# LinXueyuanStdio/LaTeX_OCR

Hardware: NVIDIA H100
Metric: formula-images/sec (train step, 128x512 px, seq<=150) (higher is better)
Workload: dtype bf16

## Files before the change

### latex_ocr_b200/csrc/lo_attention.cu

```cuda
#include <cooperative_groups.h>

#include "lo_common.cuh"
#include "lo_ptx.cuh"

namespace cg = cooperative_groups;

namespace lo {

#ifndef LO_ATT_RPW
#define LO_ATT_RPW 2
#endif
#ifndef LO_ATT_MINB
#define LO_ATT_MINB 2
#endif
#define AP_THREADS 288
#define AP_CWARPS 8
#define AP_STAGES 3
#define AP_MAXSPLIT 16


#ifdef LO_ATT_TIMING
__device__ long long* g_att_ts = nullptr;
__device__ __forceinline__ void att_ts(int k) {
  if (g_att_ts) {
    long long t;
    asm volatile("mov.u64 %0, %%globaltimer;" : "=l"(t));
    g_att_ts[((int64_t)blockIdx.y * gridDim.x + blockIdx.x) * 16 + k] = t;
  }
}
#define ATT_TS(k, cond) do { if (cond) att_ts(k); } while (0)
#else
#define ATT_TS(k, cond) do { } while (0)
#endif

__device__ __forceinline__ uint64_t make_policy(int kind) {
  return kind == 1 ? l2_policy_evict_last() : (kind == 2 ? l2_policy_evict_first() : l2_policy_evict_normal());
}

template <int ACT, bool APPROX>
__device__ __forceinline__ float att_act(float x) {
  if constexpr (ACT == 0) return fmaxf(x, 0.f);
  else if constexpr (APPROX) {
    float y;
    asm("tanh.approx.f32 %0, %1;" : "=f"(y) : "f"(x));
    return y;
  } else return tanhf(x);
}
template <int ACT>
__device__ __forceinline__ float att_dact(float pre, float post) {
  if constexpr (ACT == 0) return pre > 0.f ? 1.f : 0.f;
  else return 1.f - post * post;
}

__host__ __device__ __forceinline__ int att_rows_per_split(int R, int nsplit) { return (((R + nsplit - 1) / nsplit) + 1) & ~1; }

template <typename T, int NVA, int NVC>
struct ApCfg {
  static constexpr int CHA = NVA * 256;
  static constexpr int CHC = NVC * 256;
  static constexpr int NVM = NVA > NVC ? NVA : NVC;
  static constexpr int RPW = (sizeof(T) == 2 && NVM <= 2) ? LO_ATT_RPW : 1;
  static constexpr int ROWS = AP_CWARPS * RPW;
  static constexpr int HALF_A = ROWS * CHA;
  static constexpr int HALF_C = ROWS * CHC;
  static constexpr int STAGE_ELEMS = HALF_A + HALF_C;
  static constexpr int STAGE_BYTES = STAGE_ELEMS * (int)sizeof(T);
  static constexpr int SMEM = AP_STAGES * STAGE_BYTES + 128;
};

template <typename T, int NVA, int NVC, bool CL, int ACT, bool MK>
__global__ void __launch_bounds__(AP_THREADS, LO_ATT_MINB) attention_fwd_pipe_kernel(
    const T* __restrict__ att1, const T* __restrict__ enc, const float* __restrict__ att2, int64_t att2_stride,
    const float* __restrict__ wf, float* __restrict__ alpha, int64_t alpha_stride, float* __restrict__ ctx,
    float* __restrict__ gate_pre, int64_t gate_stride, float* __restrict__ gctx, bf16* __restrict__ gctx_bf, int R, int nsplit,
    int* __restrict__ counters, float* __restrict__ partials, int pol_enc, int pol_att1, int rpi, uint8_t* __restrict__ mask_out) {
  using C = ApCfg<T, NVA, NVC>;
  constexpr int CHA = C::CHA, CHC = C::CHC;
  extern __shared__ __align__(128) uint8_t ap_smem[];
  T* ring = reinterpret_cast<T*>(ap_smem);
  uint64_t* full_bar = reinterpret_cast<uint64_t*>(ap_smem + AP_STAGES * C::STAGE_BYTES);
  uint64_t* empty_bar = full_bar + AP_STAGES;
  float* s_e = reinterpret_cast<float*>(ap_smem + AP_STAGES * C::STAGE_BYTES + 128);
  __shared__ float s_m[AP_CWARPS], s_l[AP_CWARPS];
  __shared__ float s_scale[AP_MAXSPLIT];
  __shared__ float s_ML[2];
  __shared__ int s_last;

  const int b = blockIdx.y, sp = blockIdx.x;
  const int lane = threadIdx.x & 31, wid = threadIdx.x >> 5;
  const int rps = (R + nsplit - 1) / nsplit;
  const int r0 = sp * rps, r1 = min(R, r0 + rps);
  const int nst = r1 > r0 ? (r1 - r0 + C::ROWS - 1) / C::ROWS : 0;
  const T* a1b = att1 + (int64_t)(b / rpi) * R * CHA;
  const T* eb = enc + (int64_t)(b / rpi) * R * CHC;
  float* alb = alpha + (int64_t)b * alpha_stride;
  ATT_TS(0, threadIdx.x == 0);

  if (threadIdx.x == 0) {
    for (int s = 0; s < AP_STAGES; s++) {
      mbar_init(full_bar + s, 1);
      mbar_init(empty_bar + s, AP_CWARPS);
    }
    fence_barrier_init();
  }
  __syncthreads();
  float m = -INFINITY, l = 0.f;
  float gate_pf = 0.f;
  float acc[NVC * 8];
#pragma unroll
  for (int i = 0; i < NVC * 8; i++) acc[i] = 0.f;

  if (wid == AP_CWARPS) {
    if (lane == 0) {
      const uint64_t pe = make_policy(pol_enc), pa = make_policy(pol_att1);
      for (int i = 0; i < nst; i++) {
        const int s = i % AP_STAGES;
        const uint32_t ph = (i / AP_STAGES) & 1;
        mbar_wait(empty_bar + s, ph ^ 1);
        const int row = r0 + i * C::ROWS;
        const int rows = min(C::ROWS, r1 - row);
        const uint32_t bytes_a = (uint32_t)rows * CHA * (uint32_t)sizeof(T), bytes_c = (uint32_t)rows * CHC * (uint32_t)sizeof(T);
        T* sa = ring + (size_t)s * C::STAGE_ELEMS;
        mbar_expect_tx(full_bar + s, bytes_a + bytes_c);
        ATT_TS(6, i == 0);
        ATT_TS(7, i == nst - 1);
        if (pol_att1 == 3) bulk_g2s_nohint(sa, a1b + (int64_t)row * CHA, bytes_a, full_bar + s);
        else bulk_g2s(sa, a1b + (int64_t)row * CHA, bytes_a, full_bar + s, pa);
        if (pol_enc == 3) bulk_g2s_nohint(sa + C::HALF_A, eb + (int64_t)row * CHC, bytes_c, full_bar + s);
        else bulk_g2s(sa + C::HALF_A, eb + (int64_t)row * CHC, bytes_c, full_bar + s, pe);
      }
    }
    __syncwarp();
    pdl_wait();
  } else {
    float a2[NVA * 8], wv[NVA * 8];
#pragma unroll
    for (int j = 0; j < NVA; j++) ld8(wf + (j * 32 + lane) * 8, wv + j * 8);
    pdl_wait();
    ATT_TS(1, threadIdx.x == 0);
    pdl_trigger();
#pragma unroll
    for (int j = 0; j < NVA; j++) ld8(att2 + (int64_t)b * att2_stride + (j * 32 + lane) * 8, a2 + j * 8);
    if (CL && gate_pre && (int)threadIdx.x < (CHC + nsplit - 1) / nsplit && sp * ((CHC + nsplit - 1) / nsplit) + (int)threadIdx.x < CHC)
      gate_pf = gate_pre[(int64_t)b * gate_stride + sp * ((CHC + nsplit - 1) / nsplit) + threadIdx.x];
    ATT_TS(2, threadIdx.x == 0);
    for (int i = 0; i < nst; i++) {
      const int s = i % AP_STAGES;
      const uint32_t ph = (i / AP_STAGES) & 1;
      const int row = r0 + i * C::ROWS;
      const int rows = min(C::ROWS, r1 - row);
      mbar_wait(full_bar + s, ph);
      ATT_TS(3, threadIdx.x == 0 && i == 0);
      const uint32_t sa = smem_u32(ring + (size_t)s * C::STAGE_ELEMS);
      const uint32_t se = sa + C::HALF_A * (uint32_t)sizeof(T);
      constexpr uint32_t ES = (uint32_t)sizeof(T);
      const int ra = wid, rb = wid + AP_CWARPS;
      const bool one = ra < rows;
      const bool two = (C::RPW == 2) && (rb < rows);
      if (one) {
        float e0 = 0.f, e1 = 0.f;
        uint8_t* mrow = MK ? mask_out + (int64_t)b * ((R + 1) & ~1) * (CHA / 8) : nullptr;
#pragma unroll
        for (int j = 0; j < NVA; j++) {
          float v[8];
          lds8(sa + ((uint32_t)ra * CHA + (j * 32 + lane) * 8) * ES, v, (const T*)nullptr);
          uint32_t bits = 0;
#pragma unroll
          for (int q = 0; q < 8; q++) {
            const float pre = v[q] + a2[j * 8 + q];
            if (MK) bits = __funnelshift_l(__float_as_uint(pre), bits, 1);
            e0 = fmaf(wv[j * 8 + q], att_act<ACT, sizeof(T) == 2>(pre), e0);
          }
          if (MK) mrow[(int64_t)((row + ra) >> 1) * (CHA / 4) + (j * 32 + lane) * 2 + ((row + ra) & 1)] = (uint8_t)(~bits);
          if (two) {
            lds8(sa + ((uint32_t)rb * CHA + (j * 32 + lane) * 8) * ES, v, (const T*)nullptr);
            bits = 0;
#pragma unroll
            for (int q = 0; q < 8; q++) {
              const float pre = v[q] + a2[j * 8 + q];
              if (MK) bits = __funnelshift_l(__float_as_uint(pre), bits, 1);
              e1 = fmaf(wv[j * 8 + q], att_act<ACT, sizeof(T) == 2>(pre), e1);
            }
            if (MK) mrow[(int64_t)((row + rb) >> 1) * (CHA / 4) + (j * 32 + lane) * 2 + ((row + rb) & 1)] = (uint8_t)(~bits);
          }
        }
        e0 = warp_sum(e0);
        e1 = warp_sum(e1);
        if (lane == 0) {
          if constexpr (CL) {
            s_e[row + ra - r0] = e0;
            if (two) s_e[row + rb - r0] = e1;
          } else {
            alb[row + ra] = e0;
            if (two) alb[row + rb] = e1;
          }
        }
        const float mn = two ? fmaxf(m, fmaxf(e0, e1)) : fmaxf(m, e0);
        const float sc = expf(m - mn);
        const float p0 = expf(e0 - mn);
        const float p1 = two ? expf(e1 - mn) : 0.f;
        l = l * sc + p0 + p1;
#pragma unroll
        for (int j = 0; j < NVC; j++) {
          float u[8];
          lds8(se + ((uint32_t)ra * CHC + (j * 32 + lane) * 8) * ES, u, (const T*)nullptr);
#pragma unroll
          for (int q = 0; q < 8; q++) acc[j * 8 + q] = fmaf(p0, u[q], acc[j * 8 + q] * sc);
          if (two) {
            lds8(se + ((uint32_t)rb * CHC + (j * 32 + lane) * 8) * ES, u, (const T*)nullptr);
#pragma unroll
            for (int q = 0; q < 8; q++) acc[j * 8 + q] = fmaf(p1, u[q], acc[j * 8 + q]);
          }
        }
        m = mn;
      }
      __syncwarp();
      if (lane == 0) mbar_arrive(empty_bar + s);
    }
  }
  ATT_TS(4, threadIdx.x == 0);
  __syncthreads();
  ATT_TS(8, threadIdx.x == 0);
  float* s_acc = reinterpret_cast<float*>(ap_smem);
  if (wid < AP_CWARPS) {
    if (lane == 0) { s_m[wid] = m; s_l[wid] = l; }
#pragma unroll
    for (int j = 0; j < NVC; j++)
#pragma unroll
      for (int i = 0; i < 8; i++) s_acc[wid * CHC + (j * 32 + lane) * 8 + i] = acc[j * 8 + i];
  }
  __syncthreads();
  float M = -INFINITY;
#pragma unroll
  for (int w = 0; w < AP_CWARPS; w++) M = fmaxf(M, s_m[w]);
  float L = 0.f;
  float wsc[AP_CWARPS];
#pragma unroll
  for (int w = 0; w < AP_CWARPS; w++) {
    wsc[w] = (s_m[w] == -INFINITY) ? 0.f : expf(s_m[w] - M);
    L += s_l[w] * wsc[w];
  }
  if constexpr (CL) {
    cg::cluster_group cluster = cg::this_cluster();
    float* s_part = s_acc + AP_CWARPS * CHC;
    __shared__ float s_MLp[2];
    for (int c = threadIdx.x; c < CHC; c += AP_THREADS) {
      float t = 0.f;
#pragma unroll
      for (int w = 0; w < AP_CWARPS; w++) t = fmaf(s_acc[w * CHC + c], wsc[w], t);
      s_part[c] = t;
    }
    if (threadIdx.x == 0) { s_MLp[0] = M; s_MLp[1] = L; }
    cluster.sync();
    float Mg = -INFINITY;
    for (int q = 0; q < nsplit; q++) Mg = fmaxf(Mg, cluster.map_shared_rank(s_MLp, q)[0]);
    float Lg = 0.f;
    float scl[8];
#pragma unroll
    for (int q = 0; q < 8; q++) {
      scl[q] = 0.f;
      if (q < nsplit) {
        const float* ml = cluster.map_shared_rank(s_MLp, q);
        const float ms = ml[0];
        scl[q] = (ms == -INFINITY) ? 0.f : expf(ms - Mg);
        Lg += ml[1] * scl[q];
      }
    }
    const float invL = 1.0f / Lg;
    const int cps = (CHC + nsplit - 1) / nsplit;
    for (int c = sp * cps + threadIdx.x; c < min(CHC, (sp + 1) * cps); c += AP_THREADS) {
      float t = 0.f;
#pragma unroll
      for (int q = 0; q < 8; q++)
        if (q < nsplit) t = fmaf(cluster.map_shared_rank(s_part, q)[c], scl[q], t);
      t *= invL;
      ctx[(int64_t)b * CHC + c] = t;
      if (gate_pre) {
        const bool pf = c == sp * cps + (int)threadIdx.x && (int)threadIdx.x < AP_CWARPS * 32;
        const float g = sigmoidf_(pf ? gate_pf : gate_pre[(int64_t)b * gate_stride + c]);
        gate_pre[(int64_t)b * gate_stride + c] = g;
        gctx[(int64_t)b * CHC + c] = g * t;
        if (gctx_bf) gctx_bf[(int64_t)b * CHC + c] = __float2bfloat16_rn(g * t);
      } else if (gctx_bf) {
        gctx_bf[(int64_t)b * CHC + c] = __float2bfloat16_rn(t);
      }
    }
    for (int r = r0 + threadIdx.x; r < r1; r += AP_THREADS) alb[r] = expf(s_e[r - r0] - Mg) * invL;
    cluster.sync();
    ATT_TS(5, threadIdx.x == 0);
    return;
  }
  float* part = partials + ((int64_t)b * nsplit + sp) * (CHC + 2);
  for (int c = threadIdx.x; c < CHC; c += AP_THREADS) {
    float t = 0.f;
#pragma unroll
    for (int w = 0; w < AP_CWARPS; w++) t = fmaf(s_acc[w * CHC + c], wsc[w], t);
    part[2 + c] = t;
  }
  if (threadIdx.x == 0) { part[0] = M; part[1] = L; }
  __threadfence();
  __syncthreads();
  if (threadIdx.x == 0) {
    const int ticket = atomicAdd(counters + b, 1);
    s_last = (ticket == nsplit - 1);
    if (s_last) counters[b] = 0;
  }
  __syncthreads();
  if (!s_last) return;
  __threadfence();
  const float* pb = partials + (int64_t)b * nsplit * (CHC + 2);
  if (threadIdx.x == 0) {
    float Mg = -INFINITY;
    for (int s = 0; s < nsplit; s++) Mg = fmaxf(Mg, __ldcg(pb + (int64_t)s * (CHC + 2)));
    float Lg = 0.f;
    for (int s = 0; s < nsplit; s++) {
      const float ms = __ldcg(pb + (int64_t)s * (CHC + 2));
      const float scl = (ms == -INFINITY) ? 0.f : expf(ms - Mg);
      s_scale[s] = scl;
      Lg += __ldcg(pb + (int64_t)s * (CHC + 2) + 1) * scl;
    }
    s_ML[0] = Mg;
    s_ML[1] = 1.0f / Lg;
  }
  __syncthreads();
  const float Mg = s_ML[0], invL = s_ML[1];
  for (int c = threadIdx.x; c < CHC; c += AP_THREADS) {
    float t = 0.f;
    for (int s = 0; s < nsplit; s++) t = fmaf(__ldcg(pb + (int64_t)s * (CHC + 2) + 2 + c), s_scale[s], t);
    t *= invL;
    ctx[(int64_t)b * CHC + c] = t;
    if (gate_pre) {
      const float g = sigmoidf_(gate_pre[(int64_t)b * gate_stride + c]);
      gate_pre[(int64_t)b * gate_stride + c] = g;
      gctx[(int64_t)b * CHC + c] = g * t;
      if (gctx_bf) gctx_bf[(int64_t)b * CHC + c] = __float2bfloat16_rn(g * t);
    } else if (gctx_bf) {
      gctx_bf[(int64_t)b * CHC + c] = __float2bfloat16_rn(t);
    }
  }
  for (int r = threadIdx.x; r < R; r += AP_THREADS) alb[r] = expf(__ldcg(alb + r) - Mg) * invL;
}

template <typename T, int NVA, int NVC, bool CL, int ACT, bool DA1 = false>
__global__ void __launch_bounds__(AP_THREADS) attention_bwd_pipe_kernel(
    const T* __restrict__ att1, const T* __restrict__ enc, const float* __restrict__ att2, const float* __restrict__ gate,
    int64_t o1_stride, const float* __restrict__ wf, const float* __restrict__ alpha, int64_t alpha_stride,
    const float* __restrict__ ctx, const float* __restrict__ dgctx, int64_t dg_stride, const float* __restrict__ dreg,
    int64_t dreg_stride, const float* __restrict__ sreg, int64_t sreg_stride, float* __restrict__ de, float* __restrict__ datt2,
    float* __restrict__ dgp, int64_t dcat_stride, bf16* __restrict__ datt2_bf, bf16* __restrict__ dgp_bf,
    float* __restrict__ dctx_out, int R, int nsplit, int* __restrict__ counters, float* __restrict__ partials, int pol_enc,
    int pol_att1, float* __restrict__ dwf_part, T* __restrict__ datt1) {
  using C = ApCfg<T, NVA, NVC>;
  constexpr int CHA = C::CHA, CHC = C::CHC;
  extern __shared__ __align__(128) uint8_t ap_smem[];
  T* ring = reinterpret_cast<T*>(ap_smem);
  uint64_t* full_bar = reinterpret_cast<uint64_t*>(ap_smem + AP_STAGES * C::STAGE_BYTES);
  uint64_t* empty_bar = full_bar + AP_STAGES;
  __shared__ int s_last;
  const int b = blockIdx.y, sp = blockIdx.x;
  const int lane = threadIdx.x & 31, wid = threadIdx.x >> 5;
  const int rps = (R + nsplit - 1) / nsplit;
  const int r0 = sp * rps, r1 = min(R, r0 + rps);
  const int nst = r1 > r0 ? (r1 - r0 + C::ROWS - 1) / C::ROWS : 0;
  const T* a1b = att1 + (int64_t)b * R * CHA;
  const T* eb = enc + (int64_t)b * R * CHC;
  const float* s_wf = nullptr;
  if constexpr (DA1 && NVA > 2) {
    __shared__ __align__(16) float s_wbuf[CHA];
    for (int c = threadIdx.x; c < CHA; c += AP_THREADS) s_wbuf[c] = wf[c];
    s_wf = s_wbuf;
  }
  if (threadIdx.x == 0) {
    for (int s = 0; s < AP_STAGES; s++) {
      mbar_init(full_bar + s, 1);
      mbar_init(empty_bar + s, AP_CWARPS);
    }
    fence_barrier_init();
  }
  __syncthreads();
  float macc[NVA * 8], wacc[NVA * 8];
#pragma unroll
  for (int i = 0; i < NVA * 8; i++) { macc[i] = 0.f; wacc[i] = 0.f; }

  if (wid == AP_CWARPS) {
    if (lane == 0) {
      const uint64_t pe = make_policy(pol_enc), pa = make_policy(pol_att1);
      for (int i = 0; i < nst; i++) {
        const int s = i % AP_STAGES;
        const uint32_t ph = (i / AP_STAGES) & 1;
        mbar_wait(empty_bar + s, ph ^ 1);
        const int row = r0 + i * C::ROWS;
        const int rows = min(C::ROWS, r1 - row);
        const uint32_t bytes_a = (uint32_t)rows * CHA * (uint32_t)sizeof(T), bytes_c = (uint32_t)rows * CHC * (uint32_t)sizeof(T);
        T* sa = ring + (size_t)s * C::STAGE_ELEMS;
        mbar_expect_tx(full_bar + s, bytes_a + bytes_c);
        if (pol_att1 == 3) bulk_g2s_nohint(sa, a1b + (int64_t)row * CHA, bytes_a, full_bar + s);
        else bulk_g2s(sa, a1b + (int64_t)row * CHA, bytes_a, full_bar + s, pa);
        if (pol_enc == 3) bulk_g2s_nohint(sa + C::HALF_A, eb + (int64_t)row * CHC, bytes_c, full_bar + s);
        else bulk_g2s(sa + C::HALF_A, eb + (int64_t)row * CHC, bytes_c, full_bar + s, pe);
      }
    }
    __syncwarp();
    pdl_wait();
  } else {
    float a2[NVA * 8], dc[NVC * 8];
    float wv[NVA * 8];
    if constexpr (DA1 && NVA <= 2) {
#pragma unroll
      for (int j = 0; j < NVA; j++) ld8(wf + (j * 32 + lane) * 8, wv + j * 8);
    }
    float sdot = 0.f;
    float gv[NVC * 8], cxv[NVC * 8];
#pragma unroll
    for (int j = 0; j < NVA; j++) ld8(att2 + (int64_t)b * o1_stride + (j * 32 + lane) * 8, a2 + j * 8);
#pragma unroll
    for (int j = 0; j < NVC; j++) {
      const int c0 = (j * 32 + lane) * 8;
      if (gate) ld8(gate + (int64_t)b * o1_stride + c0, gv + j * 8);
      ld8(ctx + (int64_t)b * CHC + c0, cxv + j * 8);
    }
    const float sreg_b = sreg ? sreg[(int64_t)b * sreg_stride] : 0.f;
    pdl_wait();
    pdl_trigger();
// ... 322 lines not shown
          }
        }
        d0 = warp_sum(d0);
        d1 = warp_sum(d1);
        const float de0 = al0 * (d0 + dr0 - sall);
        const float de1 = two ? al1 * (d1 + dr1 - sall) : 0.f;
        if (lane == 0) {
          deb[row + ra] = de0;
          if (two) deb[row + rb] = de1;
        }
#pragma unroll
        for (int j = 0; j < NVA; j++) {
          const uint32_t m0 = sm[(ra >> 1) * 2 * MB + (j * 32 + lane) * 2 + (ra & 1)];
          const uint32_t m1 = two ? sm[(rb >> 1) * 2 * MB + (j * 32 + lane) * 2 + (rb & 1)] : 0u;
#pragma unroll
          for (int q = 0; q < 8; q++) {
            if (m0 & (0x80u >> q)) macc[j * 8 + q] += de0;
            if (m1 & (0x80u >> q)) macc[j * 8 + q] += de1;
          }
        }
      }
      __syncwarp();
      if (lane == 0) mbar_arrive(empty_bar + s);
    }
  }
  __syncthreads();
  float* s_acc = reinterpret_cast<float*>(ap_smem);
  float* s_part = s_acc + AP_CWARPS * CHA;
  if (wid < AP_CWARPS) {
#pragma unroll
    for (int j = 0; j < NVA; j++)
#pragma unroll
      for (int i = 0; i < 8; i++) s_acc[wid * CHA + (j * 32 + lane) * 8 + i] = macc[j * 8 + i];
  }
  __syncthreads();
  if constexpr (CL) {
    cg::cluster_group cluster = cg::this_cluster();
    for (int c = threadIdx.x; c < CHA; c += AP_THREADS) {
      float t = 0.f;
#pragma unroll
      for (int w = 0; w < AP_CWARPS; w++) t += s_acc[w * CHA + c];
      s_part[c] = t;
    }
    cluster.sync();
    const int cps = (CHA + nsplit - 1) / nsplit;
    for (int c = sp * cps + threadIdx.x; c < min(CHA, (sp + 1) * cps); c += AP_THREADS) {
      float t = 0.f;
      for (int q = 0; q < nsplit; q++) t += cluster.map_shared_rank(s_part, q)[c];
      if (dwf_part) dwf_part[(int64_t)b * CHA + c] += t * att2[(int64_t)b * o1_stride + c];
      datt2[(int64_t)b * dcat_stride + c] = t * wf[c];
      if (datt2_bf) datt2_bf[(int64_t)b * dcat_stride + c] = __float2bfloat16_rn(t * wf[c]);
    }
    cluster.sync();
    return;
  }
  float* part = partials + ((int64_t)b * nsplit + sp) * (CHA + 2);
  for (int c = threadIdx.x; c < CHA; c += AP_THREADS) {
    float t = 0.f;
#pragma unroll
    for (int w = 0; w < AP_CWARPS; w++) t += s_acc[w * CHA + c];
    part[2 + c] = t;
  }
  __threadfence();
  __syncthreads();
  if (threadIdx.x == 0) {
    const int ticket = atomicAdd(counters + b, 1);
    s_last = (ticket == nsplit - 1);
    if (s_last) counters[b] = 0;
  }
  __syncthreads();
  if (!s_last) return;
  __threadfence();
  const float* pb = partials + (int64_t)b * nsplit * (CHA + 2);
  for (int c = threadIdx.x; c < CHA; c += AP_THREADS) {
    float t = 0.f;
    for (int sidx = 0; sidx < nsplit; sidx++) t += __ldcg(pb + (int64_t)sidx * (CHA + 2) + 2 + c);
    if (dwf_part) dwf_part[(int64_t)b * CHA + c] += t * att2[(int64_t)b * o1_stride + c];
    datt2[(int64_t)b * dcat_stride + c] = t * wf[c];
    if (datt2_bf) datt2_bf[(int64_t)b * dcat_stride + c] = __float2bfloat16_rn(t * wf[c]);
  }
}

#ifndef LO_ABM_STAGES
#define LO_ABM_STAGES 3
#endif
#ifndef LO_ABM_MINB
#define LO_ABM_MINB 3
#endif
constexpr int ABM_STAGES = LO_ABM_STAGES;
constexpr int ABM_ROWS = 16;
constexpr int ABM_CH = 512;
constexpr int ABM_PITCH = ABM_CH * 2 + 16;
constexpr int ABM_ENC_BYTES = ABM_ROWS * ABM_PITCH;
constexpr int ABM_MSK_BYTES = ABM_ROWS * (ABM_CH / 8);
constexpr int ABM_STAGE_BYTES = ABM_ENC_BYTES + ABM_MSK_BYTES;
constexpr int ABM_SMEM = ABM_STAGES * ABM_STAGE_BYTES + 128 + 2 * AP_CWARPS * ABM_ROWS * 4;
static_assert(ABM_STAGE_BYTES % 128 == 0, "stage alignment");

__device__ __forceinline__ void att_ldsm_x4(uint32_t& r0, uint32_t& r1, uint32_t& r2, uint32_t& r3, uint32_t saddr) {
  asm volatile("ldmatrix.sync.aligned.m8n8.x4.shared.b16 {%0, %1, %2, %3}, [%4];" : "=r"(r0), "=r"(r1), "=r"(r2), "=r"(r3) : "r"(saddr));
}
__device__ __forceinline__ void att_mma_16816(float* c, uint32_t a0, uint32_t a1, uint32_t a2, uint32_t a3, uint32_t b0, uint32_t b1) {
  asm volatile("mma.sync.aligned.m16n8k16.row.col.f32.bf16.bf16.f32 {%0, %1, %2, %3}, {%4, %5, %6, %7}, {%8, %9}, {%0, %1, %2, %3};"
               : "+f"(c[0]), "+f"(c[1]), "+f"(c[2]), "+f"(c[3])
               : "r"(a0), "r"(a1), "r"(a2), "r"(a3), "r"(b0), "r"(b1));
}
__device__ __forceinline__ uint32_t pack_split(float x, float y, int sel) {
  const bf16 hx = __float2bfloat16_rn(x), hy = __float2bfloat16_rn(y);
  __nv_bfloat162 r;
  if (sel == 0) {
    r.x = hx; r.y = hy;
  } else {
    r.x = __float2bfloat16_rn(x - __bfloat162float(hx));
    r.y = __float2bfloat16_rn(y - __bfloat162float(hy));
  }
  return *reinterpret_cast<uint32_t*>(&r);
}

template <bool CL>
__global__ void __launch_bounds__(AP_THREADS, LO_ABM_MINB) attention_bwd_mma_kernel(
    const uint8_t* __restrict__ mask, const bf16* __restrict__ enc, const float* __restrict__ gate, int64_t o1_stride,
    const float* __restrict__ wf, const float* __restrict__ alpha, int64_t alpha_stride, const float* __restrict__ ctx,
    const float* __restrict__ dgctx, int64_t dg_stride, const float* __restrict__ dreg, int64_t dreg_stride,
    const float* __restrict__ sreg, int64_t sreg_stride, float* __restrict__ de, float* __restrict__ datt2, float* __restrict__ dgp,
    int64_t dcat_stride, bf16* __restrict__ datt2_bf, bf16* __restrict__ dgp_bf, float* __restrict__ dctx_out, int R, int nsplit,
    int* __restrict__ counters, float* __restrict__ partials, int pol_enc, const float* __restrict__ att2,
    float* __restrict__ dwf_part) {
  constexpr int CH = ABM_CH, MB = CH / 8;
  extern __shared__ __align__(128) uint8_t ap_smem[];
  uint64_t* full_bar = reinterpret_cast<uint64_t*>(ap_smem + ABM_STAGES * ABM_STAGE_BYTES);
  uint64_t* empty_bar = full_bar + ABM_STAGES;
  float* s_pd = reinterpret_cast<float*>(ap_smem + ABM_STAGES * ABM_STAGE_BYTES + 128);
  __shared__ int s_last;
  const int b = blockIdx.y, sp = blockIdx.x;
  const int lane = threadIdx.x & 31, wid = threadIdx.x >> 5;
  const int rps = att_rows_per_split(R, nsplit);
  const int r0 = sp * rps, r1 = min(R, r0 + rps);
  const int nst = r1 > r0 ? (r1 - r0 + ABM_ROWS - 1) / ABM_ROWS : 0;
  const int Rp = (R + 1) & ~1;
  ATT_TS(0, threadIdx.x == 0);
  const bf16* eb = enc + (int64_t)b * R * CH;
  const uint8_t* mb = mask + (int64_t)b * Rp * MB;
  if (threadIdx.x == 0) {
    for (int s = 0; s < ABM_STAGES; s++) {
      mbar_init(full_bar + s, 1);
      mbar_init(empty_bar + s, AP_CWARPS);
    }
    fence_barrier_init();
  }
  __syncthreads();
  const int g = lane >> 2, q = lane & 3;
  const int cps_pf = (CH + nsplit - 1) / nsplit;
  const int c_pf = sp * cps_pf + (int)threadIdx.x;
  float wf_pf = 0.f, a2_pf = 0.f;
  if (CL && (int)threadIdx.x < cps_pf && c_pf < CH) {
    wf_pf = wf[c_pf];
    if (dwf_part) a2_pf = att2[(int64_t)b * o1_stride + c_pf];
  }
  float macc[4][4];
#pragma unroll
  for (int j = 0; j < 4; j++)
#pragma unroll
    for (int i = 0; i < 4; i++) macc[j][i] = 0.f;

  if (wid == AP_CWARPS) {
    const uint64_t pe = make_policy(pol_enc), pm = l2_policy_evict_first();
    for (int i = 0; i < nst; i++) {
      const int s = i % ABM_STAGES;
      const uint32_t ph = (i / ABM_STAGES) & 1;
      const int row = r0 + i * ABM_ROWS;
// ... 56 lines not shown
        const float2 u = *reinterpret_cast<const float2*>(dgctx + (int64_t)b * dg_stride + k0);
        const float2 v = *reinterpret_cast<const float2*>(dgctx + (int64_t)b * dg_stride + k0 + 8);
        bd[s][0] = pack_split(u.x * gq[s][0], u.y * gq[s][1], g);
        bd[s][1] = pack_split(v.x * gq[s][2], v.y * gq[s][3], g);
      }
    }
#pragma unroll
    for (int j = 0; j < 2; j++) {
      const int c0 = (j * 32 + lane) * 8;
      float dg[8], gp[8], dc[8];
      ld8(dgctx + (int64_t)b * dg_stride + c0, dg);
#pragma unroll
      for (int i = 0; i < 8; i++) {
        const float gi = gate ? gv[j * 8 + i] : 1.f;
        dc[i] = dg[i] * gi;
        sdot = fmaf(dc[i], cxv[j * 8 + i], sdot);
        gp[i] = dg[i] * cxv[j * 8 + i] * gi * (1.f - gi);
      }
      if (sp == 0 && wid == 0) {
        if (dgp) st8(dgp + (int64_t)b * dcat_stride + c0, gp);
        if (dgp_bf) st8(dgp_bf + (int64_t)b * dcat_stride + c0, gp);
        if (dctx_out) st8(dctx_out + (int64_t)b * CH + c0, dc);
      }
    }
    const float sall = warp_sum(sdot) + sreg_b;
    ATT_TS(2, threadIdx.x == 0);
    const uint32_t ring = smem_u32(ap_smem);
    const uint32_t a_off = (uint32_t)((lane & 7) + ((lane >> 3) & 1) * 8) * ABM_PITCH + (uint32_t)(64 * wid + (lane >> 4) * 8) * 2u;
    const uint32_t m_off = ABM_ENC_BYTES + (uint32_t)q * 2u * MB + (uint32_t)(8 * wid + g) * 2u;
    asm volatile("bar.sync 1, 256;" ::: "memory");
    for (int i = 0; i < nst; i++) {
      const int s = i % ABM_STAGES;
      const uint32_t ph = (i / ABM_STAGES) & 1;
      const int row = r0 + i * ABM_ROWS;
      const int rows = min(ABM_ROWS, r1 - row);
      const float al = rr < rows ? s_al[i * ABM_ROWS + rr] : 0.f, dr = rr < rows ? s_dr[i * ABM_ROWS + rr] : 0.f;
      mbar_wait(full_bar + s, ph);
      ATT_TS(3, threadIdx.x == 0 && i == 0);
      const uint32_t sb = ring + (uint32_t)s * ABM_STAGE_BYTES;
      float d4[4] = {0.f, 0.f, 0.f, 0.f};
#pragma unroll
      for (int k = 0; k < 4; k++) {
        uint32_t a0, a1, a2, a3;
        att_ldsm_x4(a0, a1, a2, a3, sb + a_off + k * 32);
        att_mma_16816(d4, a0, a1, a2, a3, bd[k][0], bd[k][1]);
      }
      const uint32_t u_lo = *reinterpret_cast<const uint16_t*>(ap_smem + (size_t)s * ABM_STAGE_BYTES + m_off);
      const uint32_t u_hi = *reinterpret_cast<const uint16_t*>(ap_smem + (size_t)s * ABM_STAGE_BYTES + m_off + 4 * 2 * MB);
      const uint32_t mw = __byte_perm(u_lo, u_hi, 0x5140);
      float* pdw = s_pd + (i & 1) * (AP_CWARPS * ABM_ROWS);
      if (q == 0) {
        pdw[wid * ABM_ROWS + g] = d4[0] + d4[1];
        pdw[wid * ABM_ROWS + g + 8] = d4[2] + d4[3];
      }
      __syncwarp();
      if (lane == 0) mbar_arrive(empty_bar + s);
      asm volatile("bar.sync 1, 256;" ::: "memory");
      float dsum = 0.f;
#pragma unroll
      for (int w = 0; w < AP_CWARPS; w++) dsum += pdw[w * ABM_ROWS + rr];
      const float dev = rr < rows ? al * (dsum + dr - sall) : 0.f;
      if (wid == (i & 7) && lane < rows) deb[row + lane] = dev;
      const float v0 = __shfl_sync(0xffffffffu, dev, 2 * q), v1 = __shfl_sync(0xffffffffu, dev, 2 * q + 1);
      const float v2 = __shfl_sync(0xffffffffu, dev, 2 * q + 8), v3 = __shfl_sync(0xffffffffu, dev, 2 * q + 9);
      uint32_t bm0 = 0u, bm1 = 0u;
      if (g < 2) {
        bm0 = pack_split(v0, v1, g);
        bm1 = pack_split(v2, v3, g);
      }
#pragma unroll
      for (int j = 0; j < 4; j++) {
        uint32_t af[4];
#pragma unroll
        for (int ii = 0; ii < 4; ii++) {
          const int h = ii & 1, rs = ii >> 1;
          const int sh = 14 - (8 * rs + 7 - (2 * j + h));
          af[ii] = (sh >= 0 ? (mw << sh) : (mw >> (-sh))) & 0x40004000u;
        }
        att_mma_16816(macc[j], af[0], af[1], af[2], af[3], bm0, bm1);
      }
    }
  }
  ATT_TS(4, threadIdx.x == 0);
  __syncthreads();
  ATT_TS(8, threadIdx.x == 0);
  float* s_part = reinterpret_cast<float*>(ap_smem);
  if (wid < AP_CWARPS && q == 0) {
#pragma unroll
    for (int j = 0; j < 4; j++) {
      s_part[64 * wid + 8 * g + 2 * j] = 0.5f * (macc[j][0] + macc[j][1]);
      s_part[64 * wid + 8 * g + 2 * j + 1] = 0.5f * (macc[j][2] + macc[j][3]);
    }
  }
  __syncthreads();
  if constexpr (CL) {
    cg::cluster_group cluster = cg::this_cluster();
    const float dwf_pf = dwf_part && (int)threadIdx.x < cps_pf && c_pf < CH ? dwf_part[(int64_t)b * CH + c_pf] : 0.f;
    cluster.sync();
    const int cps = (CH + nsplit - 1) / nsplit;
    float* s_sum = s_part + CH;
    for (int c = sp * cps + threadIdx.x; c < min(CH, (sp + 1) * cps); c += AP_THREADS) {
      float t = 0.f;
      for (int qq = 0; qq < nsplit; qq++) t += cluster.map_shared_rank(s_part, qq)[c];
      s_sum[c - sp * cps] = t;
    }
    cl_arrive_release();
    for (int c = sp * cps + threadIdx.x; c < min(CH, (sp + 1) * cps); c += AP_THREADS) {
      const float t = s_sum[c - sp * cps];
      const bool pf = c == c_pf;
      const float wfc = pf ? wf_pf : wf[c];
      if (dwf_part)
        dwf_part[(int64_t)b * CH + c] = (pf ? dwf_pf : dwf_part[(int64_t)b * CH + c]) + t * (pf ? a2_pf : att2[(int64_t)b * o1_stride + c]);
      datt2[(int64_t)b * dcat_stride + c] = t * wfc;
      if (datt2_bf) datt2_bf[(int64_t)b * dcat_stride + c] = __float2bfloat16_rn(t * wfc);
    }
    cl_wait_acquire();
    ATT_TS(5, threadIdx.x == 0);
    return;
  }
  float* part = partials + ((int64_t)b * nsplit + sp) * (CH + 2);
  for (int c = threadIdx.x; c < CH; c += AP_THREADS) part[2 + c] = s_part[c];
  __threadfence();
  __syncthreads();
  if (threadIdx.x == 0) {
    const int ticket = atomicAdd(counters + b, 1);
    s_last = (ticket == nsplit - 1);
    if (s_last) counters[b] = 0;
  }
  __syncthreads();
  if (!s_last) return;
  __threadfence();
  const float* pb = partials + (int64_t)b * nsplit * (CH + 2);
  for (int c = threadIdx.x; c < CH; c += AP_THREADS) {
    float t = 0.f;
    for (int sidx = 0; sidx < nsplit; sidx++) t += __ldcg(pb + (int64_t)sidx * (CH + 2) + 2 + c);
    if (dwf_part) dwf_part[(int64_t)b * CH + c] += t * att2[(int64_t)b * o1_stride + c];
    datt2[(int64_t)b * dcat_stride + c] = t * wf[c];
    if (datt2_bf) datt2_bf[(int64_t)b * dcat_stride + c] = __float2bfloat16_rn(t * wf[c]);
  }
}

int att_pipe_splits(int B, int hint = 0) {
  if (g_opt_att_nsplit > 0) return g_opt_att_nsplit > AP_MAXSPLIT ? AP_MAXSPLIT : g_opt_att_nsplit;
  if (hint > 0) return hint > 8 ? 8 : hint;
  int s = (LO_NUM_SMS * LO_ATT_MINB) / B;
  if (s < 1) s = 1;
  if (s > AP_MAXSPLIT) s = AP_MAXSPLIT;
  if (g_opt_att_cluster && s > 8) s = 8;
  return s;
}

static cudaAccessPolicyWindow g_att_window{};

static inline bool att_pdl_ok(int abi) { return !abi || g_opt_att_abi_pdl; }

template <typename... KArgs, typename... Args>
static cudaError_t launch_att(void (*kernel)(KArgs...), dim3 grid, size_t smem, int cluster_x, cudaStream_t st, bool pdl, Args... args) {
  cudaLaunchConfig_t cfg{};
  cfg.gridDim = grid;
  cfg.blockDim = dim3(AP_THREADS);
  cfg.dynamicSmemBytes = smem;
  cfg.stream = st;
  cudaLaunchAttribute attr[3];
  int n = 0;
  if (g_att_window.num_bytes) {
    attr[n].id = cudaLaunchAttributeAccessPolicyWindow;
    attr[n].val.accessPolicyWindow = g_att_window;
    n++;
  }
  if (g_opt_pdl && pdl) {
    attr[n].id = cudaLaunchAttributeProgrammaticStreamSerialization;
    attr[n].val.programmaticStreamSerializationAllowed = 1;
    n++;
  }
  if (cluster_x > 1) {
    attr[n].id = cudaLaunchAttributeClusterDimension;
    attr[n].val.clusterDim.x = cluster_x;
    attr[n].val.clusterDim.y = 1;
    attr[n].val.clusterDim.z = 1;
    n++;
  }
  cfg.attrs = attr;
  cfg.numAttrs = n;
  return cudaLaunchKernelEx(&cfg, kernel, KArgs(args)...);
}

static inline bool use_cluster(int ns, int R) {
  return g_opt_att_cluster && ns >= 2 && ns <= 8 && ((R + ns - 1) / ns) * 4 <= 16 * 1024;
}

template <typename T, int NVA, int NVC, int ACT, bool MK>
static int fwd_launch_m(const AttFwdArgs& x, cudaStream_t st) {
  using C = ApCfg<T, NVA, NVC>;
  constexpr int SM_MAX = C::SMEM + 16 * 1024;
  static bool attr = false;
  if (!attr) {
    LO_CUDA(cudaFuncSetAttribute(attention_fwd_pipe_kernel<T, NVA, NVC, false, ACT, MK>, cudaFuncAttributeMaxDynamicSharedMemorySize, C::SMEM));
    LO_CUDA(cudaFuncSetAttribute(attention_fwd_pipe_kernel<T, NVA, NVC, true, ACT, MK>, cudaFuncAttributeMaxDynamicSharedMemorySize, SM_MAX));
    attr = true;
  }
  const int ns = att_pipe_splits(x.B, x.nsplit_hint);
  const int rpi = x.rows_per_img > 1 ? x.rows_per_img : 1;
  if (use_cluster(ns, x.R)) {
    const size_t smem = C::SMEM + (size_t)((x.R + ns - 1) / ns) * 4;
    LO_CUDA(launch_att(attention_fwd_pipe_kernel<T, NVA, NVC, true, ACT, MK>, dim3(ns, x.B), smem, ns, st, att_pdl_ok(x.abi), (const T*)x.att1, (const T*)x.enc,
                       x.att2, x.att2_stride, x.wf, x.alpha, x.alpha_stride, x.ctx, x.gate_pre, x.gate_stride, x.gctx, x.gctx_bf, x.R, ns,
                       (int*)x.work, (float*)((char*)x.work + 4096), g_opt_att_policy_enc, g_opt_att_policy_att1, rpi, x.mask_out));
  } else {
    LO_CUDA(launch_att(attention_fwd_pipe_kernel<T, NVA, NVC, false, ACT, MK>, dim3(ns, x.B), (size_t)C::SMEM, 1, st, att_pdl_ok(x.abi), (const T*)x.att1,
                       (const T*)x.enc, x.att2, x.att2_stride, x.wf, x.alpha, x.alpha_stride, x.ctx, x.gate_pre, x.gate_stride, x.gctx,
                       x.gctx_bf, x.R, ns, (int*)x.work, (float*)((char*)x.work + 4096), g_opt_att_policy_enc, g_opt_att_policy_att1, rpi,
                       x.mask_out));
  }
  LO_LAUNCH_OK();
  return LO_OK;
}

template <typename T, int NVA, int NVC, int ACT>
static int fwd_launch_a(const AttFwdArgs& x, cudaStream_t st) {
  if constexpr (ACT == 0) {
    if (x.mask_out) return fwd_launch_m<T, NVA, NVC, ACT, true>(x, st);
  }
  return fwd_launch_m<T, NVA, NVC, ACT, false>(x, st);
}

template <typename T, int NVA, int NVC>
static int fwd_launch(const AttFwdArgs& x, cudaStream_t st) {
  return x.act == 1 ? fwd_launch_a<T, NVA, NVC, 1>(x, st) : fwd_launch_a<T, NVA, NVC, 0>(x, st);
}

template <typename T>
static int fwd_dispatch(const AttFwdArgs& x, int C, cudaStream_t st) {
  const int A = x.a_ch > 0 ? x.a_ch : C;
  if (A == 256 && C == 512) return fwd_launch<T, 1, 2>(x, st);
  if (A != C) return fail(LO_EINVAL, "%s: attention width pair (%ld, %ld) not instantiated", __func__, A, C);
  if (C == 256) return fwd_launch<T, 1, 1>(x, st);
  if (C == 512) return fwd_launch<T, 2, 2>(x, st);
  return fwd_launch<T, 4, 4>(x, st);
}
int attention_fwd_pipe(const AttFwdArgs& x, int dt, int C, cudaStream_t st) {
  return dt == LO_F32 ? fwd_dispatch<float>(x, C, st) : fwd_dispatch<bf16>(x, C, st);
}

template <typename T, int NVA, int NVC, int ACT>
static int bwd_launch_a(const AttBwdArgs& x, cudaStream_t st) {
  using C = ApCfg<T, NVA, NVC>;
  static bool attr = false;
  if (!attr) {
    LO_CUDA(cudaFuncSetAttribute(attention_bwd_pipe_kernel<T, NVA, NVC, false, ACT>, cudaFuncAttributeMaxDynamicSharedMemorySize, C::SMEM));
    LO_CUDA(cudaFuncSetAttribute(attention_bwd_pipe_kernel<T, NVA, NVC, true, ACT>, cudaFuncAttributeMaxDynamicSharedMemorySize, C::SMEM));
    attr = true;
  }
  const int ns = att_pipe_splits(x.B, x.nsplit_hint);
  if (x.datt1) {
    if constexpr (ACT == 0) {
      LO_CHECK_ARG(!x.mask_in, "d att1 is computed from att1, not from the mask bits");
      static bool attr_d = false;
      if (!attr_d) {
        LO_CUDA(cudaFuncSetAttribute(attention_bwd_pipe_kernel<T, NVA, NVC, false, ACT, true>, cudaFuncAttributeMaxDynamicSharedMemorySize, C::SMEM));
        LO_CUDA(cudaFuncSetAttribute(attention_bwd_pipe_kernel<T, NVA, NVC, true, ACT, true>, cudaFuncAttributeMaxDynamicSharedMemorySize, C::SMEM));
        attr_d = true;
      }
      const int nsd = (x.ordered_dwf && x.dwf_part && !use_cluster(ns, x.R)) ? 1 : ns;
#define LO_BWDD_ARGS                                                                                                             \
  (const T*)x.att1, (const T*)x.enc, x.att2, x.gate, x.o1_stride, x.wf, x.alpha, x.alpha_stride, x.ctx, x.dgctx, x.dg_stride, x.dreg, \
      x.dreg_stride, x.sreg, x.sreg_stride, x.de, x.datt2, x.dgp, x.dcat_stride, x.datt2_bf, x.dgp_bf, x.dctx_out, x.R, nsd,      \
      (int*)x.work, (float*)((char*)x.work + 4096), g_opt_att_policy_enc, g_opt_att_policy_att1, x.dwf_part, (T*)x.datt1
      if (use_cluster(nsd, x.R)) {
        LO_CUDA(launch_att(attention_bwd_pipe_kernel<T, NVA, NVC, true, ACT, true>, dim3(nsd, x.B), (size_t)C::SMEM, nsd, st, att_pdl_ok(x.abi),
                           LO_BWDD_ARGS));
      } else {
        LO_CUDA(launch_att(attention_bwd_pipe_kernel<T, NVA, NVC, false, ACT, true>, dim3(nsd, x.B), (size_t)C::SMEM, 1, st, att_pdl_ok(x.abi),
                           LO_BWDD_ARGS));
      }
#undef LO_BWDD_ARGS
      LO_LAUNCH_OK();
      return LO_OK;
    }
    return fail(LO_EINVAL, "%s: d att1 is only produced for the ReLU score", __func__);
  }
  if constexpr (ACT == 0 && sizeof(T) == 2 && NVA == 2 && NVC == 2)
  if (x.mask_in && g_opt_att_bwd_mma && att_rows_per_split(x.R, ns) <= 2048) {
    static bool attr_t = false;
    if (!attr_t) {
      LO_CUDA(cudaFuncSetAttribute(attention_bwd_mma_kernel<false>, cudaFuncAttributeMaxDynamicSharedMemorySize, ABM_SMEM + 2048 * 8));
      LO_CUDA(cudaFuncSetAttribute(attention_bwd_mma_kernel<true>, cudaFuncAttributeMaxDynamicSharedMemorySize, ABM_SMEM + 2048 * 8));
      attr_t = true;
    }
#define LO_BWDT_ARGS                                                                                                                  \
  x.mask_in, (const bf16*)x.enc, x.gate, x.o1_stride, x.wf, x.alpha, x.alpha_stride, x.ctx, x.dgctx, x.dg_stride, x.dreg,            \
      x.dreg_stride, x.sreg, x.sreg_stride, x.de, x.datt2, x.dgp, x.dcat_stride, x.datt2_bf, x.dgp_bf, x.dctx_out, x.R, ns,           \
      (int*)x.work, (float*)((char*)x.work + 4096), 2, x.att2, x.dwf_part
    const size_t smem_t = (size_t)ABM_SMEM + (size_t)att_rows_per_split(x.R, ns) * 8;
    if (use_cluster(ns, x.R)) {
      LO_CUDA(launch_att(attention_bwd_mma_kernel<true>, dim3(ns, x.B), smem_t, ns, st, att_pdl_ok(x.abi), LO_BWDT_ARGS));
    } else {
      LO_CUDA(launch_att(attention_bwd_mma_kernel<false>, dim3(ns, x.B), smem_t, 1, st, att_pdl_ok(x.abi), LO_BWDT_ARGS));
    }
#undef LO_BWDT_ARGS
    LO_LAUNCH_OK();
    return LO_OK;
  }
  if constexpr (ACT == 0) if (x.mask_in) {
    using CM = ApmCfg<T, NVA, NVC>;
    static bool attr_m = false;
    if (!attr_m) {
      LO_CUDA(cudaFuncSetAttribute(attention_bwd_mask_kernel<T, NVA, NVC, false>, cudaFuncAttributeMaxDynamicSharedMemorySize, CM::SMEM));
      LO_CUDA(cudaFuncSetAttribute(attention_bwd_mask_kernel<T, NVA, NVC, true>, cudaFuncAttributeMaxDynamicSharedMemorySize, CM::SMEM));
      attr_m = true;
    }
#define LO_BWDM_ARGS                                                                                                                  \
  x.mask_in, (const T*)x.enc, x.gate, x.o1_stride, x.wf, x.alpha, x.alpha_stride, x.ctx, x.dgctx, x.dg_stride, x.dreg, x.dreg_stride, \
      x.sreg, x.sreg_stride, x.de, x.datt2, x.dgp, x.dcat_stride, x.datt2_bf, x.dgp_bf, x.dctx_out, x.R, ns, (int*)x.work,           \
      (float*)((char*)x.work + 4096), g_opt_att_policy_enc, x.att2, x.dwf_part
    if (use_cluster(ns, x.R)) {
      LO_CUDA(launch_att(attention_bwd_mask_kernel<T, NVA, NVC, true>, dim3(ns, x.B), (size_t)CM::SMEM, ns, st, att_pdl_ok(x.abi), LO_BWDM_ARGS));
    } else {
      LO_CUDA(launch_att(attention_bwd_mask_kernel<T, NVA, NVC, false>, dim3(ns, x.B), (size_t)CM::SMEM, 1, st, att_pdl_ok(x.abi), LO_BWDM_ARGS));
    }
#undef LO_BWDM_ARGS
    LO_LAUNCH_OK();
    return LO_OK;
  }
#define LO_BWD_ARGS                                                                                                              \
  (const T*)x.att1, (const T*)x.enc, x.att2, x.gate, x.o1_stride, x.wf, x.alpha, x.alpha_stride, x.ctx, x.dgctx, x.dg_stride, x.dreg, \
      x.dreg_stride, x.sreg, x.sreg_stride, x.de, x.datt2, x.dgp, x.dcat_stride, x.datt2_bf, x.dgp_bf, x.dctx_out, x.R, ns,       \
      (int*)x.work, (float*)((char*)x.work + 4096), g_opt_att_policy_enc, g_opt_att_policy_att1, x.dwf_part, (T*)nullptr
  if (use_cluster(ns, x.R)) {
    LO_CUDA(launch_att(attention_bwd_pipe_kernel<T, NVA, NVC, true, ACT>, dim3(ns, x.B), (size_t)C::SMEM, ns, st, att_pdl_ok(x.abi), LO_BWD_ARGS));
  } else {
    LO_CUDA(launch_att(attention_bwd_pipe_kernel<T, NVA, NVC, false, ACT>, dim3(ns, x.B), (size_t)C::SMEM, 1, st, att_pdl_ok(x.abi), LO_BWD_ARGS));
  }
#undef LO_BWD_ARGS
  LO_LAUNCH_OK();
  return LO_OK;
}

template <typename T, int NVA, int NVC>
static int bwd_launch(const AttBwdArgs& x, cudaStream_t st) {
  return x.act == 1 ? bwd_launch_a<T, NVA, NVC, 1>(x, st) : bwd_launch_a<T, NVA, NVC, 0>(x, st);
}

template <typename T>
static int bwd_dispatch(const AttBwdArgs& x, int C, cudaStream_t st) {
  const int A = x.a_ch > 0 ? x.a_ch : C;
  if (A == 256 && C == 512) return bwd_launch<T, 1, 2>(x, st);
  if (A != C) return fail(LO_EINVAL, "%s: attention width pair (%ld, %ld) not instantiated", __func__, A, C);
  if (C == 256) return bwd_launch<T, 1, 1>(x, st);
  if (C == 512) return bwd_launch<T, 2, 2>(x, st);
  return bwd_launch<T, 4, 4>(x, st);
}
int attention_bwd_pipe(const AttBwdArgs& x, int dt, int C, cudaStream_t st) {
  return dt == LO_F32 ? bwd_dispatch<float>(x, C, st) : bwd_dispatch<bf16>(x, C, st);
}

}

namespace lo { extern long long* g_tc_dbg; }
extern "C" int lo_debug_buffer(void* p) {
  lo::g_tc_dbg = (long long*)p;
  LO_TRY(lo::cl_set_ts((long long*)p));
  LO_TRY(lo::sk_set_ts((long long*)p));
#ifdef LO_ATT_TIMING
  long long* q = (long long*)p;
  LO_CUDA(cudaMemcpyToSymbol(lo::g_att_ts, &q, sizeof(q)));
#endif
  return LO_OK;
}

extern "C" int lo_set_l2_window(const void* base, int64_t bytes, float hit_ratio, void* stream) {
  int dev = 0, max_persist = 0, max_window = 0;
  LO_CUDA(cudaGetDevice(&dev));
  LO_CUDA(cudaDeviceGetAttribute(&max_persist, cudaDevAttrMaxPersistingL2CacheSize, dev));
  LO_CUDA(cudaDeviceGetAttribute(&max_window, cudaDevAttrMaxAccessPolicyWindowSize, dev));
  cudaStreamAttrValue v{};
  if (bytes <= 0 || !base) {
    v.accessPolicyWindow.num_bytes = 0;
// ... 18 lines not shown
```

Baseline: 2097.

## Prefetch split-merge operands and choose cluster launch by grid residency

```diff
diff --git a/latex_ocr_b200/csrc/lo_attention.cu b/latex_ocr_b200/csrc/lo_attention.cu
--- a/latex_ocr_b200/csrc/lo_attention.cu
+++ b/latex_ocr_b200/csrc/lo_attention.cu
@@ -1,4 +1,7 @@
 #include <cooperative_groups.h>
+
+#include <mutex>
+#include <vector>
 
 #include "lo_common.cuh"
 #include "lo_ptx.cuh"
@@ -82,8 +85,7 @@
   uint64_t* empty_bar = full_bar + AP_STAGES;
   float* s_e = reinterpret_cast<float*>(ap_smem + AP_STAGES * C::STAGE_BYTES + 128);
   __shared__ float s_m[AP_CWARPS], s_l[AP_CWARPS];
-  __shared__ float s_scale[AP_MAXSPLIT];
-  __shared__ float s_ML[2];
+  __shared__ float s_msplit[AP_MAXSPLIT], s_lsplit[AP_MAXSPLIT];
   __shared__ int s_last;
 
   const int b = blockIdx.y, sp = blockIdx.x;
@@ -219,6 +221,15 @@
     }
   }
   ATT_TS(4, threadIdx.x == 0);
+  constexpr int NCI = (CHC + AP_THREADS - 1) / AP_THREADS;
+  float gpf[NCI];
+  if constexpr (!CL) {
+#pragma unroll
+    for (int k = 0; k < NCI; k++) {
+      const int c = threadIdx.x + k * AP_THREADS;
+      gpf[k] = (gate_pre && c < CHC) ? gate_pre[(int64_t)b * gate_stride + c] : 0.f;
+    }
+  }
   __syncthreads();
   ATT_TS(8, threadIdx.x == 0);
   float* s_acc = reinterpret_cast<float*>(ap_smem);
@@ -306,39 +317,69 @@
     if (s_last) counters[b] = 0;
   }
   __syncthreads();
-  if (!s_last) return;
+  if (!s_last) {
+    ATT_TS(5, threadIdx.x == 0);
+    return;
+  }
   __threadfence();
+  ATT_TS(9, threadIdx.x == 0);
   const float* pb = partials + (int64_t)b * nsplit * (CHC + 2);
-  if (threadIdx.x == 0) {
-    float Mg = -INFINITY;
-    for (int s = 0; s < nsplit; s++) Mg = fmaxf(Mg, __ldcg(pb + (int64_t)s * (CHC + 2)));
-    float Lg = 0.f;
-    for (int s = 0; s < nsplit; s++) {
-      const float ms = __ldcg(pb + (int64_t)s * (CHC + 2));
-      const float scl = (ms == -INFINITY) ? 0.f : expf(ms - Mg);
-      s_scale[s] = scl;
-      Lg += __ldcg(pb + (int64_t)s * (CHC + 2) + 1) * scl;
-    }
-    s_ML[0] = Mg;
-    s_ML[1] = 1.0f / Lg;
-  }
-  __syncthreads();
-  const float Mg = s_ML[0], invL = s_ML[1];
-  for (int c = threadIdx.x; c < CHC; c += AP_THREADS) {
-    float t = 0.f;
-    for (int s = 0; s < nsplit; s++) t = fmaf(__ldcg(pb + (int64_t)s * (CHC + 2) + 2 + c), s_scale[s], t);
-    t *= invL;
-    ctx[(int64_t)b * CHC + c] = t;
-    if (gate_pre) {
-      const float g = sigmoidf_(gate_pre[(int64_t)b * gate_stride + c]);
-      gate_pre[(int64_t)b * gate_stride + c] = g;
-      gctx[(int64_t)b * CHC + c] = g * t;
-      if (gctx_bf) gctx_bf[(int64_t)b * CHC + c] = __float2bfloat16_rn(g * t);
-    } else if (gctx_bf) {
-      gctx_bf[(int64_t)b * CHC + c] = __float2bfloat16_rn(t);
-    }
-  }
-  for (int r = threadIdx.x; r < R; r += AP_THREADS) alb[r] = expf(__ldcg(alb + r) - Mg) * invL;
+  constexpr int PS = 8;
+  constexpr int RB = 4;
+  if ((int)threadIdx.x < nsplit) {
+    s_msplit[threadIdx.x] = __ldcg(pb + (int64_t)threadIdx.x * (CHC + 2));
+    s_lsplit[threadIdx.x] = __ldcg(pb + (int64_t)threadIdx.x * (CHC + 2) + 1);
+  }
+  float pv[PS], ev[RB];
+  auto load_parts = [&](int c) {
+#pragma unroll
+    for (int s = 0; s < PS; s++) pv[s] = s < nsplit ? __ldcg(pb + (int64_t)s * (CHC + 2) + 2 + c) : 0.f;
+  };
+  if ((int)threadIdx.x < CHC) load_parts(threadIdx.x);
+#pragma unroll
+  for (int k = 0; k < RB; k++) {
+    const int r = threadIdx.x + k * AP_THREADS;
+    ev[k] = r < R ? __ldcg(alb + r) : 0.f;
+  }
+  __syncthreads();
+  float Mg = -INFINITY;
+  for (int s = 0; s < nsplit; s++) Mg = fmaxf(Mg, s_msplit[s]);
+  auto split_scale = [&](int s) {
+    const float ms = s_msplit[s];
+    return (ms == -INFINITY) ? 0.f : expf(ms - Mg);
+  };
+  float Lg = 0.f;
+  for (int s = 0; s < nsplit; s++) Lg += s_lsplit[s] * split_scale(s);
+  const float invL = 1.0f / Lg;
+#pragma unroll
+  for (int k = 0; k < NCI; k++) {
+    const int c = threadIdx.x + k * AP_THREADS;
+    if (c < CHC) {
+      if (k > 0) load_parts(c);
+      float t = 0.f;
+#pragma unroll
+      for (int s = 0; s < PS; s++)
+        if (s < nsplit) t = fmaf(pv[s], split_scale(s), t);
+      for (int s = PS; s < nsplit; s++) t = fmaf(__ldcg(pb + (int64_t)s * (CHC + 2) + 2 + c), split_scale(s), t);
+      t *= invL;
+      ctx[(int64_t)b * CHC + c] = t;
+      if (gate_pre) {
+        const float g = sigmoidf_(gpf[k]);
+        gate_pre[(int64_t)b * gate_stride + c] = g;
+        gctx[(int64_t)b * CHC + c] = g * t;
+        if (gctx_bf) gctx_bf[(int64_t)b * CHC + c] = __float2bfloat16_rn(g * t);
+      } else if (gctx_bf) {
+        gctx_bf[(int64_t)b * CHC + c] = __float2bfloat16_rn(t);
+      }
+    }
+  }
+#pragma unroll
+  for (int k = 0; k < RB; k++) {
+    const int r = threadIdx.x + k * AP_THREADS;
+    if (r < R) alb[r] = expf(ev[k] - Mg) * invL;
+  }
+  for (int r = threadIdx.x + RB * AP_THREADS; r < R; r += AP_THREADS) alb[r] = expf(__ldcg(alb + r) - Mg) * invL;
+  ATT_TS(5, threadIdx.x == 0);
 }
 
 template <typename T, int NVA, int NVC, bool CL, int ACT, bool DA1 = false>
@@ -827,10 +868,10 @@
 }
 
 #ifndef LO_ABM_STAGES
-#define LO_ABM_STAGES 3
+#define LO_ABM_STAGES 5
 #endif
 #ifndef LO_ABM_MINB
-#define LO_ABM_MINB 3
+#define LO_ABM_MINB 2
 #endif
 constexpr int ABM_STAGES = LO_ABM_STAGES;
 constexpr int ABM_ROWS = 16;
@@ -1053,6 +1094,17 @@
     }
   }
   ATT_TS(4, threadIdx.x == 0);
+  constexpr int NCB = (CH + AP_THREADS - 1) / AP_THREADS;
+  float wf_t[NCB], a2_t[NCB], dwf_t[NCB];
+  if constexpr (!CL) {
+#pragma unroll
+    for (int k = 0; k < NCB; k++) {
+      const int c = threadIdx.x + k * AP_THREADS;
+      wf_t[k] = c < CH ? wf[c] : 0.f;
+      a2_t[k] = (dwf_part && c < CH) ? att2[(int64_t)b * o1_stride + c] : 0.f;
+      dwf_t[k] = (dwf_part && c < CH) ? dwf_part[(int64_t)b * CH + c] : 0.f;
+    }
+  }
   __syncthreads();
   ATT_TS(8, threadIdx.x == 0);
   float* s_part = reinterpret_cast<float*>(ap_smem);
@@ -1099,16 +1151,32 @@
     if (s_last) counters[b] = 0;
   }
   __syncthreads();
-  if (!s_last) return;
+  if (!s_last) {
+    ATT_TS(5, threadIdx.x == 0);
+    return;
+  }
   __threadfence();
+  ATT_TS(9, threadIdx.x == 0);
   const float* pb = partials + (int64_t)b * nsplit * (CH + 2);
-  for (int c = threadIdx.x; c < CH; c += AP_THREADS) {
-    float t = 0.f;
-    for (int sidx = 0; sidx < nsplit; sidx++) t += __ldcg(pb + (int64_t)sidx * (CH + 2) + 2 + c);
-    if (dwf_part) dwf_part[(int64_t)b * CH + c] += t * att2[(int64_t)b * o1_stride + c];
-    datt2[(int64_t)b * dcat_stride + c] = t * wf[c];
-    if (datt2_bf) datt2_bf[(int64_t)b * dcat_stride + c] = __float2bfloat16_rn(t * wf[c]);
-  }
+  constexpr int PS = 8;
+#pragma unroll
+  for (int k = 0; k < NCB; k++) {
+    const int c = threadIdx.x + k * AP_THREADS;
+    if (c < CH) {
+      float pv[PS];
+#pragma unroll
+      for (int s = 0; s < PS; s++) pv[s] = s < nsplit ? __ldcg(pb + (int64_t)s * (CH + 2) + 2 + c) : 0.f;
+      float t = 0.f;
+#pragma unroll
+      for (int s = 0; s < PS; s++)
+        if (s < nsplit) t += pv[s];
+      for (int s = PS; s < nsplit; s++) t += __ldcg(pb + (int64_t)s * (CH + 2) + 2 + c);
+      if (dwf_part) dwf_part[(int64_t)b * CH + c] = dwf_t[k] + t * a2_t[k];
+      datt2[(int64_t)b * dcat_stride + c] = t * wf_t[k];
+      if (datt2_bf) datt2_bf[(int64_t)b * dcat_stride + c] = __float2bfloat16_rn(t * wf_t[k]);
+    }
+  }
+  ATT_TS(5, threadIdx.x == 0);
 }
 
 int att_pipe_splits(int B, int hint = 0) {
@@ -1160,6 +1228,31 @@
   return g_opt_att_cluster && ns >= 2 && ns <= 8 && ((R + ns - 1) / ns) * 4 <= 16 * 1024;
 }
 
+static int att_resident_ctas(const void* kernel, size_t smem) {
+  struct Entry { int dev; const void* k; size_t smem; int ctas; };
+  static std::mutex mu;
+  static std::vector<Entry> cache;
+  int dev = 0;
+  if (cudaGetDevice(&dev) != cudaSuccess) return 0;
+  std::lock_guard<std::mutex> lock(mu);
+  for (const Entry& e : cache)
+    if (e.dev == dev && e.k == kernel && e.smem == smem) return e.ctas;
+  int per_sm = 0, sms = 0;
+  if (cudaOccupancyMaxActiveBlocksPerMultiprocessor(&per_sm, kernel, AP_THREADS, smem) != cudaSuccess ||
+      cudaDeviceGetAttribute(&sms, cudaDevAttrMultiProcessorCount, dev) != cudaSuccess) {
+    cudaGetLastError();
+    return 0;
+  }
+  cache.push_back({dev, kernel, smem, per_sm * sms});
+  return per_sm * sms;
+}
+
+static bool att_grid_cluster(const void* free_kernel, size_t free_smem, int ns, int B, int R) {
+  if (!use_cluster(ns, R)) return false;
+  if (g_opt_att_cluster != 1) return true;
+  return att_resident_ctas(free_kernel, free_smem) < ns * B;
+}
+
 template <typename T, int NVA, int NVC, int ACT, bool MK>
 static int fwd_launch_m(const AttFwdArgs& x, cudaStream_t st) {
   using C = ApCfg<T, NVA, NVC>;
@@ -1172,7 +1265,7 @@
   }
   const int ns = att_pipe_splits(x.B, x.nsplit_hint);
   const int rpi = x.rows_per_img > 1 ? x.rows_per_img : 1;
-  if (use_cluster(ns, x.R)) {
+  if (att_grid_cluster((const void*)attention_fwd_pipe_kernel<T, NVA, NVC, false, ACT, MK>, (size_t)C::SMEM, ns, x.B, x.R)) {
     const size_t smem = C::SMEM + (size_t)((x.R + ns - 1) / ns) * 4;
     LO_CUDA(launch_att(attention_fwd_pipe_kernel<T, NVA, NVC, true, ACT, MK>, dim3(ns, x.B), smem, ns, st, att_pdl_ok(x.abi), (const T*)x.att1, (const T*)x.enc,
                        x.att2, x.att2_stride, x.wf, x.alpha, x.alpha_stride, x.ctx, x.gate_pre, x.gate_stride, x.gctx, x.gctx_bf, x.R, ns,
@@ -1263,7 +1356,7 @@
       x.dreg_stride, x.sreg, x.sreg_stride, x.de, x.datt2, x.dgp, x.dcat_stride, x.datt2_bf, x.dgp_bf, x.dctx_out, x.R, ns,           \
       (int*)x.work, (float*)((char*)x.work + 4096), 2, x.att2, x.dwf_part
     const size_t smem_t = (size_t)ABM_SMEM + (size_t)att_rows_per_split(x.R, ns) * 8;
-    if (use_cluster(ns, x.R)) {
+    if (att_grid_cluster((const void*)attention_bwd_mma_kernel<false>, smem_t, ns, x.B, x.R)) {
       LO_CUDA(launch_att(attention_bwd_mma_kernel<true>, dim3(ns, x.B), smem_t, ns, st, att_pdl_ok(x.abi), LO_BWDT_ARGS));
     } else {
       LO_CUDA(launch_att(attention_bwd_mma_kernel<false>, dim3(ns, x.B), smem_t, 1, st, att_pdl_ok(x.abi), LO_BWDT_ARGS));
```

Result: faster. 2245, median of 6 (+7.1%).
